# helemanc/audio-based-lyrics-matching

Measured on NVIDIA B200. Metric: similarity+MAP eval Gpairs/s at 1/2/4/8 B200 (roofline frac); MAP parity, higher is better.
Workload: dtype f16 tensor-core hi/lo split x3, f32 accumulate

## Files before the change

audio-based-lyrics-matching_b200/csrc/eval_sym_epilogue.cuh:

```cuda
#pragma once
#include "gemm_core.cuh"

namespace wealy {

struct EvalSymParams {
  const float4* lvl;
  const uint2* cinfo;
  const int* s_c;
  const int* s_i;
  const float* thr;
  unsigned int* hist;
  const unsigned char* dirty;
  int n_col_tiles;
  int n_row_blocks;
  unsigned int total_pairs;
  const float* beta;
  float* tk_val;
  int* tk_idx;
  int* tk_cnt;
  int tk_cap;
};

__device__ __forceinline__ unsigned bit_transpose32(unsigned x, int lane) {
#pragma unroll
  for (int s = 16; s >= 1; s >>= 1) {
    const unsigned mask = s == 16 ? 0x0000ffffu : s == 8 ? 0x00ff00ffu : s == 4 ? 0x0f0f0f0fu : s == 2 ? 0x33333333u : 0x55555555u;
    const unsigned y = __shfl_xor_sync(0xffffffffu, x, s);
    x = (lane & s) ? ((x & ~mask) | ((y >> s) & mask)) : ((x & mask) | ((y << s) & ~mask));
  }
  return x;
}

template <int kLv, int kQueueCapT = 256, int kCachePairsT = 4096, bool kTopk = false>
struct EvalSymEpi {
  static_assert(kLv >= 2 && kLv <= 4, "2..4 register levels");
  static_assert(!kTopk || kLv <= 3, "the top-k bound of the columns rides in the 4th threshold slot");
  using Params = EvalSymParams;
  static constexpr int kQueueCap = kQueueCapT;
  static constexpr int kCachePairs = kCachePairsT;
  static constexpr unsigned kGlobal = 0x80000000u;
  static constexpr int kOffQx = kQueueCap * 4;
  static constexpr int kOffQn = kOffQx + kQueueCap * 4;
  static constexpr int kStageCols = 16;
  static constexpr int kOffStage = kOffQn + kQueueCap * 4;
  static constexpr int kWarpScratchBytes = kOffStage + kStageCols * 32 * 4;
  static constexpr int kColSlots = 3;
  static constexpr int kLvlBytes = kTileN * 16;
  static constexpr int kInfoBytes = kTileN * 8;
  static constexpr int kColSlotBytes = kLvlBytes + kInfoBytes;
  static constexpr int kOffColSlots = (kCachePairs * 4 + 15) / 16 * 16;
  static constexpr int kCtaScratchBytes = kOffColSlots + kColSlots * kColSlotBytes;

  __device__ static __forceinline__ void col_bulk_src(const Params& p, int t, const void*& s0, const void*& s1) {
    s0 = p.lvl + (size_t)t * kTileN;
    s1 = p.cinfo + (size_t)t * kTileN;
  }

  struct RowState {
    float t[kLv];
    unsigned rc[kLv - 1];
    unsigned rinfo;
    int rpc;
    int qc, qi;
    unsigned off;
    int qn;
    int n_cached;
    unsigned base;
    int row_glob, row_ok, dirty;
    float beta;
  };

  __device__ static __forceinline__ float* q_val(const EpiCtx& c) { return reinterpret_cast<float*>(c.warp_scratch); }
  __device__ static __forceinline__ unsigned* q_idx(const EpiCtx& c) { return reinterpret_cast<unsigned*>(c.warp_scratch + kOffQx); }
  __device__ static __forceinline__ int* q_len(const EpiCtx& c) { return reinterpret_cast<int*>(c.warp_scratch + kOffQn); }
  __device__ static __forceinline__ float* stage(const EpiCtx& c) { return reinterpret_cast<float*>(c.warp_scratch + kOffStage); }
  __device__ static __forceinline__ float* thr_s(const EpiCtx& c) { return reinterpret_cast<float*>(c.cta_scratch); }

  __device__ static __forceinline__ float lvl_of(const float4& v, int j) {
    return j == 0 ? v.x : (j == 1 ? v.y : (j == 2 ? v.z : v.w));
  }

  __device__ static __forceinline__ void row_begin(const Params& p, RowState& st, int row, int part,
                                                   const GemmShape& sh, const EpiCtx& ctx) {
    (void)part;
    const float inf = __int_as_float(0x7f800000);
#pragma unroll
    for (int j = 0; j < kLv; ++j) st.t[j] = inf;
#pragma unroll
    for (int j = 0; j < kLv - 1; ++j) st.rc[j] = 0u;
    st.qc = st.qi = 0;
    st.off = 0u;
    st.beta = inf;
    int cnt = 0;
    const int srow = spread_sorted_of(row);
    st.row_ok = srow < sh.m_rows;
    if (st.row_ok) {
      const float4 v = __ldg(p.lvl + row);
#pragma unroll
      for (int j = 0; j < kLv; ++j) st.t[j] = lvl_of(v, j);
      const uint2 ci = __ldg(p.cinfo + row);
      st.off = ci.x;
      cnt = (int)ci.y;
      st.qc = __ldg(p.s_c + srow);
      st.qi = __ldg(p.s_i + srow);
      if constexpr (kTopk) st.beta = __ldg(p.beta + row);
    }
    st.qn = 0;
    st.row_glob = row;
    st.dirty = 0;
    st.base = __ldg(p.cinfo + ctx.row_base).x;
    const unsigned end = (ctx.row_base + ctx.row_span < sh.m_rows) ? __ldg(p.cinfo + ctx.row_base + ctx.row_span).x : p.total_pairs;
    const unsigned total = end - st.base;
    st.n_cached = (int)(total < (unsigned)kCachePairs ? total : (unsigned)kCachePairs);
    float* ts = thr_s(ctx);
    for (int i = ctx.tid; i < st.n_cached; i += ctx.nthreads) ts[i] = __ldg(p.thr + st.base + i);
    const unsigned rel = st.off - st.base;
    const bool cached = st.row_ok && rel + (unsigned)cnt <= (unsigned)st.n_cached;
    st.rinfo = cached ? (rel + kLv) : (kGlobal | (st.off + kLv));
    st.rpc = cnt - kLv;
    ptx::named_barrier_sync(1, ctx.nthreads);
  }

  __device__ static __forceinline__ int warp_incl_scan(int v, int lane) {
#pragma unroll
    for (int o = 1; o < 32; o <<= 1) {
      const int t = __shfl_up_sync(0xffffffffu, v, o);
      if (lane >= o) v += t;
    }
    return v;
  }

  struct Ent {
    float s;
    unsigned idx;
    int len;
    int cand;
    bool on;
    const float* tp;
  };
  __device__ static __forceinline__ void fetch(const Params& p, const EpiCtx& ctx, Ent& en, int r, int end) {
    en.on = r < end;
    en.s = en.on ? q_val(ctx)[r] : 0.f;
    en.idx = en.on ? q_idx(ctx)[r] : 0u;
    const int raw = en.on ? q_len(ctx)[r] : 0;
    en.len = max(raw, 0);
    en.cand = kTopk ? -1 - raw : -1;
    en.tp = (en.idx & kGlobal) ? (p.thr + (en.idx & ~kGlobal)) : (thr_s(ctx) + en.idx);
  }
  __device__ static __forceinline__ void count(const Params& p, const RowState& st, const EpiCtx& ctx, const Ent& en,
                                               int lb, int lane) {
    (void)ctx; (void)lane;
    if constexpr (kTopk) {
      if (en.cand >= 0) {
        if (en.on) {
          const int pos = atomicAdd(p.tk_cnt + en.idx, 1);
          if (pos < p.tk_cap) {
            p.tk_val[(size_t)en.idx * p.tk_cap + pos] = en.s;
            p.tk_idx[(size_t)en.idx * p.tk_cap + pos] = en.cand;
          }
        }
        return;
      }
    }
    const bool glob = (en.idx & kGlobal) != 0u;
    const unsigned slot = (en.idx & ~kGlobal) - 1u + (unsigned)lb + (glob ? 0u : st.base);
    if (en.on) atomicAdd(p.hist + slot, 1u);
  }

  __device__ static __forceinline__ void drain(const Params& p, RowState& st, const EpiCtx& ctx) {
    if (st.qn == 0) return;
    const int lane = (int)ptx::lane_id();
    __syncwarp();
    const int end = st.qn;
    for (int r0 = 0; r0 < end; r0 += 64) {
      Ent a, b;
      fetch(p, ctx, a, r0 + lane, end);
      fetch(p, ctx, b, r0 + 32 + lane, end);
      int loa = 0, hia = a.len, lob = 0, hib = b.len;
      while (loa < hia || lob < hib) {
        if (loa < hia) {
          const int mid = (loa + hia) >> 1;
          if (a.tp[mid] < a.s) loa = mid + 1; else hia = mid;
        }
        if (lob < hib) {
          const int mid = (lob + hib) >> 1;
          if (b.tp[mid] < b.s) lob = mid + 1; else hib = mid;
        }
      }
      count(p, st, ctx, a, loa, lane);
      if (r0 + 32 < end) count(p, st, ctx, b, lob, lane);
    }
    __syncwarp();
    st.qn = 0;
  }

  __device__ static __forceinline__ void push(const RowState& st, const EpiCtx& ctx, const uint32_t (&acc)[32], unsigned mr,
                                              unsigned mcq, const uint2* cinf, int pos, unsigned tkr = 0u, unsigned tkc = 0u,
                                              int col0 = 0) {
    float* qv = q_val(ctx);
    unsigned* qx = q_idx(ctx);
    int* ql = q_len(ctx);
    float* stg = stage(ctx) + (ptx::lane_id());
#pragma unroll
    for (int h = 0; h < 32 / kStageCols; ++h) {
      const unsigned sel = ((1u << kStageCols) - 1u) << (h * kStageCols);
      if (!__any_sync(0xffffffffu, ((mr | mcq | tkr | tkc) & sel) != 0u)) continue;
#pragma unroll
      for (int e = 0; e < kStageCols; ++e) stg[e * 32] = __uint_as_float(acc[h * kStageCols + e]);
      unsigned m = mr & sel;
      while (m) {
        const int e = __ffs(m) - 1;
        m &= m - 1;
        qv[pos] = stg[(e - h * kStageCols) * 32];
        qx[pos] = st.rinfo;
        ql[pos] = st.rpc;
        ++pos;
      }
      m = mcq & sel;
      while (m) {
        const int e = __ffs(m) - 1;
        m &= m - 1;
        const uint2 c = cinf[e];
        qv[pos] = stg[(e - h * kStageCols) * 32];
        qx[pos] = kGlobal | (c.x + kLv);
        ql[pos] = (int)c.y - kLv;
        ++pos;
      }
      if constexpr (kTopk) {
        m = tkr & sel;
        while (m) {
          const int e = __ffs(m) - 1;
          m &= m - 1;
          qv[pos] = stg[(e - h * kStageCols) * 32];
          qx[pos] = (unsigned)st.row_glob;
          ql[pos] = -1 - (col0 + e);
          ++pos;
        }
        m = tkc & sel;
        while (m) {
          const int e = __ffs(m) - 1;
          m &= m - 1;
          qv[pos] = stg[(e - h * kStageCols) * 32];
          qx[pos] = (unsigned)(col0 + e);
          ql[pos] = -1 - st.row_glob;
          ++pos;
        }
      }
      __syncwarp();
    }
  }

  __device__ static __forceinline__ void tile_begin(const Params& p, RowState& st, const GemmShape& sh,
                                                    const EpiCtx& ctx, int t) {
    (void)sh;
    st.dirty = 0;
    for (int rbi = ctx.row_base / kTileM; rbi < (ctx.row_base + ctx.row_span) / kTileM; ++rbi)
      st.dirty |= rbi < p.n_row_blocks ? (int)__ldg(p.dirty + (size_t)rbi * p.n_col_tiles + t) : 1;
  }

  __device__ static __forceinline__ void chunk32(const Params& p, RowState& st, int row, int col0,
                                                 const uint32_t (&acc)[32], const GemmShape& sh, const EpiCtx& ctx) {
    constexpr unsigned kFull = 0xffffffffu;
    const int lane = (int)ptx::lane_id();
    (void)row;
    const float4* lv = reinterpret_cast<const float4*>(ctx.col_slot) + (col0 & (kTileN - 1));
    const uint2* cinf = reinterpret_cast<const uint2*>(ctx.col_slot + kLvlBytes) + (col0 & (kTileN - 1));

    unsigned m[kLv], mc[kLv];
    unsigned tkr = 0u, tkc = 0u;
#pragma unroll
    for (int j = 0; j < kLv; ++j) m[j] = mc[j] = 0u;
#pragma unroll
    for (int e = 0; e < 32; ++e) {
      const float s = __uint_as_float(acc[e]);
      const float4 c = lv[e];
#pragma unroll
      for (int j = 0; j < kLv; ++j) {
        m[j] |= (s > st.t[j]) ? (1u << e) : 0u;
        mc[j] |= (s > lvl_of(c, j)) ? (1u << e) : 0u;
      }
      if constexpr (kTopk) {
        tkr |= (s > st.beta) ? (1u << e) : 0u;
        tkc |= (s > c.w) ? (1u << e) : 0u;
      }
    }
    if (st.dirty) {
      const int scol = spread_sorted_of(col0 + lane);
      const bool ok = scol < sh.n_cols;
      const int cc = ok ? __ldg(p.s_c + scol) : 0;
      const int ci = ok ? __ldg(p.s_i + scol) : 0;
      unsigned valid = 0u, validk = 0u;
#pragma unroll
      for (int e = 0; e < 32; ++e) {
        const int cce = __shfl_sync(kFull, cc, e);
        const int cie = __shfl_sync(kFull, ci, e);
        const int oke = __shfl_sync(kFull, (int)ok, e);
        valid |= (oke && cce != st.qc && cie != st.qi) ? (1u << e) : 0u;
        if constexpr (kTopk) validk |= (oke && cie != st.qi) ? (1u << e) : 0u;
      }
      const int d = st.row_glob - col0;
      const unsigned above = d < 0 ? 0xffffffffu : (d >= 31 ? 0u : (0xffffffffu << (d + 1)));
      valid &= above;
      validk &= above;
      if (!st.row_ok) valid = validk = 0u;
#pragma unroll
      for (int j = 0; j < kLv; ++j) {
        m[j] &= valid;
        mc[j] &= valid;
      }
      tkr &= validk;
      tkc &= validk;
    }
    if constexpr (kTopk) {
      if (!__any_sync(kFull, (m[0] | mc[0] | tkr | tkc) != 0u)) return;
    } else {
      if (!__any_sync(kFull, (m[0] | mc[0]) != 0u)) return;
    }

#pragma unroll
    for (int j = 0; j < kLv - 1; ++j) st.rc[j] += (unsigned)__popc(m[j] ^ m[j + 1]);
    if (__any_sync(kFull, (mc[0] ^ mc[kLv - 1]) != 0u)) {
      const unsigned coff = cinf[lane].x;
#pragma unroll
      for (int j = 0; j < kLv - 1; ++j) {
        const unsigned n = (unsigned)__popc(bit_transpose32(mc[j] ^ mc[j + 1], lane));
        if (n != 0u) atomicAdd(p.hist + coff + j, n);
      }
    }

    const unsigned dr = m[kLv - 1], dc = mc[kLv - 1];
    if (!__any_sync(kFull, (dr | dc | tkr | tkc) != 0u)) return;
    const int mine = __popc(dr) + __popc(dc) + __popc(tkr) + __popc(tkc);
    const int incl = warp_incl_scan(mine, lane);
    const int total = __shfl_sync(kFull, incl, 31);
    if (st.qn + total > kQueueCap) drain(p, st, ctx);
    if (total <= kQueueCap) {
      push(st, ctx, acc, dr, dc, cinf, st.qn + incl - mine, tkr, tkc, col0);
      st.qn += total;
    } else {
      constexpr int kBatchCols = kQueueCap / (kTopk ? 128 : 64);
      static_assert(kBatchCols >= 1 && 32 % kBatchCols == 0, "queue capacity: 64 (128 with top-k) .. 2048, a power of two");
#pragma unroll 1
      for (int g = 0; g < 32 / kBatchCols; ++g) {
        const unsigned sel = ((1u << kBatchCols) - 1u) << (kBatchCols * g);
        const int mine_g = __popc(dr & sel) + __popc(dc & sel) + __popc(tkr & sel) + __popc(tkc & sel);
        const int incl_g = warp_incl_scan(mine_g, lane);
        push(st, ctx, acc, dr & sel, dc & sel, cinf, incl_g - mine_g, tkr & sel, tkc & sel, col0);
        st.qn = __shfl_sync(kFull, incl_g, 31);
        drain(p, st, ctx);
      }
    }
  }

  __device__ static __forceinline__ void tile_end(const Params& p, RowState& st, const GemmShape&, const EpiCtx& ctx) {
    if (st.qn >= kQueueCap / 2) drain(p, st, ctx);
  }

  __device__ static __forceinline__ void row_end(const Params& p, RowState& st, int row, int part,
                                                 const GemmShape& sh, const EpiCtx& ctx) {
    (void)row; (void)part; (void)sh;
    drain(p, st, ctx);
    if (st.row_ok) {
#pragma unroll
      for (int j = 0; j < kLv - 1; ++j)
        if (st.rc[j] != 0u) atomicAdd(p.hist + st.off + j, st.rc[j]);
    }
    ptx::named_barrier_sync(1, ctx.nthreads);
  }
};

}
```

audio-based-lyrics-matching_b200/csrc/gemm_core2.cuh:

```cuda
#pragma once
#include "gemm_core.cuh"

namespace wealy {

template <int kPasses, int kBlockK, int kStages>
struct PairSmem {
  static constexpr int kSwizzle = kBlockK * 2;
  static constexpr int kTileBytes = kTileM * kBlockK * 2;
  static constexpr int kPlanes = kPasses == 3 ? 2 : 1;
  static constexpr int kStageBytes = kPlanes * 2 * kTileBytes;
  static constexpr int kBarBytes = 512;
  static constexpr int kCore = kStages * kStageBytes + kBarBytes;
  static constexpr int total(int epi_warps, int scratch_per_warp, int cta_scratch) {
    return kCore + epi_warps * scratch_per_warp + cta_scratch + 1024;
  }
};

template <class Epi, int kPasses, int kBlockK, int kEpiWarps, int kStages, bool kDynChunks = false>
__global__ void __cluster_dims__(2, 1, 1) __launch_bounds__(64 + kEpiWarps * 32, 1)
gemm_pair_kernel(const __grid_constant__ GemmTmaps tmaps, const GemmShape shape, const typename Epi::Params ep) {
  using SM = PairSmem<kPasses, kBlockK, kStages>;
  using CS = ColSlotTraits<Epi>;
  constexpr int kHalves = kEpiWarps / 4;
  constexpr int kColSlots = CS::kSlots;
#ifdef WEALY_LATE_RELEASE
  constexpr bool kEarlyRelease = false;
#else
  constexpr bool kEarlyRelease = true;
#endif
  static_assert(kEpiWarps == 8 || kEpiWarps == 12, "8 or 12 epilogue warps (2 or 3 per TMEM lane quadrant)");
  static_assert(kColSlots > 0 || !kDynChunks, "dynamic chunk claiming belongs to the symmetric evaluation epilogue");

  extern __shared__ uint8_t smem_raw[];
  uint8_t* smem = smem_raw + ((1024u - (ptx::smem_u32(smem_raw) & 1023u)) & 1023u);
  uint8_t* bar_base = smem + kStages * SM::kStageBytes;
  uint64_t* full_bar = reinterpret_cast<uint64_t*>(bar_base);
  uint64_t* empty_bar = full_bar + kStages;
  uint64_t* tmem_full = empty_bar + kStages;
  uint64_t* tmem_empty = tmem_full + 2;
  uint64_t* unit_full = tmem_empty + 2;
  uint64_t* unit_empty = unit_full + 2;
  uint64_t* col_full = unit_empty + 2;
  uint64_t* col_empty = col_full + (kColSlots > 0 ? kColSlots : 1);
  int* unit_slot = reinterpret_cast<int*>(col_empty + (kColSlots > 0 ? kColSlots : 1));
  uint32_t* tmem_slot = reinterpret_cast<uint32_t*>(unit_slot + 2);
  int* chunk_ctr = reinterpret_cast<int*>(tmem_slot + 2);
  static_assert((2 * kStages + 8 + 2 * (kColSlots > 0 ? kColSlots : 1)) * 8 + 16 + 32 <= SM::kBarBytes, "barrier area");
  constexpr int kChunksPerTile = kTileN / kChunkCols;
  uint8_t* scratch_base = bar_base + SM::kBarBytes;
  uint8_t* col_slots = scratch_base + kEpiWarps * Epi::kWarpScratchBytes + CS::kOffset;

  const int warp_idx = __shfl_sync(0xffffffffu, (int)(threadIdx.x >> 5), 0);
  const int lane = (int)ptx::lane_id();
  const uint32_t cta_rank = ptx::cluster_ctarank();
  const bool leader = cta_rank == 0;

  if (warp_idx == 0 && lane == 0) {
    ptx::prefetch_tensormap(&tmaps.a_hi);
    ptx::prefetch_tensormap(&tmaps.b_hi);
    if (kPasses == 3) {
      ptx::prefetch_tensormap(&tmaps.a_lo);
      ptx::prefetch_tensormap(&tmaps.b_lo);
    }
    for (int s = 0; s < kStages; ++s) {
      ptx::mbar_init(&full_bar[s], 1);
      ptx::mbar_init(&empty_bar[s], 1);
    }
    for (int a = 0; a < 2; ++a) {
      ptx::mbar_init(&tmem_full[a], 1);
      ptx::mbar_init(&tmem_empty[a], kDynChunks ? 2 * 4 * kChunksPerTile : 2 * kEpiWarps);
      ptx::mbar_init(&unit_full[a], 1);
      ptx::mbar_init(&unit_empty[a], 2 * kEpiWarps + 2);
    }
    for (int c = 0; c < kColSlots; ++c) {
      ptx::mbar_init(&col_full[c], 1);
      ptx::mbar_init(&col_empty[c], kDynChunks ? 4 * kChunksPerTile : kEpiWarps);
    }
    for (int k = 0; k < 8; ++k) chunk_ctr[k] = 0;
    ptx::fence_mbar_init();
  }
  if (warp_idx == 1) ptx::tmem_alloc_pair<512>(tmem_slot);
  ptx::tc_fence_before_sync();
  ptx::cluster_sync_all();
  ptx::tc_fence_after_sync();
  const uint32_t tmem_base = *tmem_slot;

  const int n_units = shape.n_row_blocks * shape.n_col_chunks;

  auto unit_tiles_c = [&](int u, int& S, int& t0, int& t1, int& chunk) {
    decode_unit(shape, u, chunk, S);
    t1 = min((chunk + 1) * shape.tiles_per_chunk, shape.n_col_tiles);
    t0 = shape.sym ? max(chunk * shape.tiles_per_chunk, S) : chunk * shape.tiles_per_chunk;
  };
  auto unit_tiles = [&](int u, int& S, int& t0, int& t1) {
    int chunk;
    unit_tiles_c(u, S, t0, t1, chunk);
  };

  if (warp_idx == 0) {
    if (lane == 0) {
      int stage = 0;
      uint32_t phase = 0;
      int us = 0;
      uint32_t uphase = 0;
      int cs = 0;
      uint32_t cphase = 0;
      const uint32_t leader_full0 = ptx::map_to_cta(&full_bar[0], 0);
      const uint32_t peer_unit_full0 = ptx::map_to_cta(&unit_full[0], 1);
      const uint32_t peer_unit_slot0 = ptx::map_to_cta(&unit_slot[0], 1);
      const uint32_t leader_unit_empty0 = ptx::map_to_cta(&unit_empty[0], 0);
      const uint32_t peer_chunk_ctr0 = ptx::map_to_cta(&chunk_ctr[0], 1);
      while (true) {
        int u;
        if (leader) {
          ptx::mbar_wait_cluster(&unit_empty[us], uphase ^ 1u);
          u = atomicAdd(shape.unit_counter, 1);
          if (u >= n_units) u = -1;
          unit_slot[us] = u;
          ptx::st_cluster_u32(peer_unit_slot0 + 4u * us, (uint32_t)u);
          if constexpr (kDynChunks) {
            for (int k = 0; k < 4; ++k) {
              chunk_ctr[us * 4 + k] = 0;
              ptx::st_cluster_u32(peer_chunk_ctr0 + 4u * (us * 4 + k), 0u);
            }
          }
          ptx::mbar_arrive(&unit_full[us]);
          ptx::mbar_arrive_cluster(peer_unit_full0 + 8u * us);
        } else {
          ptx::mbar_wait_cluster(&unit_full[us], uphase);
          u = unit_slot[us];
          ptx::mbar_arrive_cluster_relaxed(leader_unit_empty0 + 8u * us);
        }
        if (++us == 2) { us = 0; uphase ^= 1u; }
        if (u < 0) break;
        int rb, t0, t1;
        unit_tiles(u, rb, t0, t1);
        for (int t = t0; t < t1; ++t) {
          if constexpr (kColSlots > 0) {
            ptx::mbar_wait(&col_empty[cs], cphase ^ 1u);
            const void *s0, *s1;
            Epi::col_bulk_src(ep, t, s0, s1);
            uint8_t* dst = col_slots + cs * CS::kBytes;
            ptx::mbar_expect_tx(&col_full[cs], CS::kBytes);
            ptx::bulk_load(dst, s0, Epi::kLvlBytes, &col_full[cs]);
            ptx::bulk_load(dst + Epi::kLvlBytes, s1, CS::kBytes - Epi::kLvlBytes, &col_full[cs]);
            if (++cs == kColSlots) { cs = 0; cphase ^= 1u; }
          }
          for (int kb = 0; kb < shape.k_blocks; ++kb) {
            ptx::mbar_wait_cluster(&empty_bar[stage], phase ^ 1u);
            uint8_t* st = smem + stage * SM::kStageBytes;
            if (leader) ptx::mbar_expect_tx(&full_bar[stage], 2 * SM::kStageBytes);
            const uint32_t fb = leader_full0 + 8u * stage;
            const int brow = t * kTileN + (int)cta_rank * kTileM;
            const int arow = (shape.sym & 2) ? rb * 2 * kTileM + (int)cta_rank : rb * 2 * kTileM + (int)cta_rank * kTileM;
            ptx::tma_load_2d_pair(st, &tmaps.a_hi, fb, kb * kBlockK, arow, ptx::kEvictLast);
            ptx::tma_load_2d_pair(st + SM::kPlanes * SM::kTileBytes, &tmaps.b_hi, fb, kb * kBlockK, brow, ptx::kEvictNormal);
            if (kPasses == 3) {
              ptx::tma_load_2d_pair(st + SM::kTileBytes, &tmaps.a_lo, fb, kb * kBlockK, arow, ptx::kEvictLast);
              ptx::tma_load_2d_pair(st + 3 * SM::kTileBytes, &tmaps.b_lo, fb, kb * kBlockK, brow, ptx::kEvictNormal);
            }
            if (++stage == kStages) { stage = 0; phase ^= 1u; }
          }
        }
      }
    }
  } else if (warp_idx == 1) {
    if (lane == 0 && leader) {
      constexpr uint32_t idesc = ptx::make_idesc_f16(2 * kTileM, kTileN, false);
      int stage = 0;
      uint32_t phase = 0;
      int acc = 0;
      uint32_t acc_phase = 0;
      int us = 0;
      uint32_t uphase = 0;
#ifdef WEALY_PROFILE_WAITS
      long long w_unit = 0, w_acc = 0, w_full = 0, n_tiles_done = 0;
      const long long t_begin = clock64();
#define WEALY_TIMED(var, stmt) { const long long _t = clock64(); stmt; var += clock64() - _t; }
#else
#define WEALY_TIMED(var, stmt) stmt;
#endif
      while (true) {
        WEALY_TIMED(w_unit, ptx::mbar_wait(&unit_full[us], uphase))
        const int u = unit_slot[us];
        ptx::mbar_arrive(&unit_empty[us]);
        if (++us == 2) { us = 0; uphase ^= 1u; }
        if (u < 0) break;
        int rb, t0, t1;
        unit_tiles(u, rb, t0, t1);
        for (int t = t0; t < t1; ++t) {
          WEALY_TIMED(w_acc, ptx::mbar_wait_cluster(&tmem_empty[acc], acc_phase ^ 1u))
          ptx::tc_fence_after_sync();
#ifdef WEALY_PROFILE_WAITS
          ++n_tiles_done;
#endif
          const uint32_t d_tmem = tmem_base + (uint32_t)(acc * kTileN);
          for (int kb = 0; kb < shape.k_blocks; ++kb) {
            WEALY_TIMED(w_full, ptx::mbar_wait_cluster(&full_bar[stage], phase))
            ptx::tc_fence_after_sync();
            const uint32_t st = ptx::smem_u32(smem + stage * SM::kStageBytes);
            const uint64_t a_hi = ptx::make_smem_desc<SM::kSwizzle>(st);
            const uint64_t a_lo = ptx::make_smem_desc<SM::kSwizzle>(st + SM::kTileBytes);
            const uint64_t b_hi = ptx::make_smem_desc<SM::kSwizzle>(st + SM::kPlanes * SM::kTileBytes);
            const uint64_t b_lo = ptx::make_smem_desc<SM::kSwizzle>(st + 3 * SM::kTileBytes);
#pragma unroll
            for (int kk = 0; kk < kBlockK / kUmmaK; ++kk) {
              const uint64_t adv = (uint64_t)((kk * kUmmaK * 2) >> 4);
              ptx::umma_f16_pair(d_tmem, a_hi + adv, b_hi + adv, idesc, (uint32_t)((kb | kk) != 0));
              if (kPasses == 3) {
                ptx::umma_f16_pair(d_tmem, a_hi + adv, b_lo + adv, idesc, 1u);
                ptx::umma_f16_pair(d_tmem, a_lo + adv, b_hi + adv, idesc, 1u);
              }
            }
            ptx::umma_commit_pair(&empty_bar[stage]);
            if (kb == shape.k_blocks - 1) ptx::umma_commit_pair(&tmem_full[acc]);
            if (++stage == kStages) { stage = 0; phase ^= 1u; }
          }
          if (++acc == 2) { acc = 0; acc_phase ^= 1u; }
        }
      }
#ifdef WEALY_PROFILE_WAITS
      if ((blockIdx.x % 37) == 0)
        printf("wealy waits: cta %d tiles %lld total %lld cyc | wait unit %lld acc(epilogue) %lld full(tma) %lld\n", (int)blockIdx.x,
               n_tiles_done, clock64() - t_begin, w_unit, w_acc, w_full);
#endif
    }
  } else {
    const int ew = warp_idx - 2;
    const int quad = warp_idx & 3;
    const int half = ew >> 2;
    const int row_in_tile = quad * 32 + lane;
    int acc = 0;
    uint32_t acc_phase = 0;
    int us = 0;
    uint32_t uphase = 0;
    int cs = 0;
    uint32_t cphase = 0;
    const uint32_t leader_unit_empty0 = ptx::map_to_cta(&unit_empty[0], 0);
    const uint32_t leader_tmem_empty0 = ptx::map_to_cta(&tmem_empty[0], 0);
    unsigned tile_seq = 0;
    int pending_slot = -1;
    while (true) {
      ptx::mbar_wait_cluster_warp(&unit_full[us], uphase);
      const int u = unit_slot[us];
      const int us_claim = us;
      __syncwarp();
      if constexpr (kDynChunks) {
        if (pending_slot >= 0 && lane == 0) ptx::mbar_arrive_cluster_relaxed(leader_unit_empty0 + 8u * pending_slot);
        pending_slot = us;
      } else {
        if (lane == 0) ptx::mbar_arrive_cluster_relaxed(leader_unit_empty0 + 8u * us);
      }
      if (++us == 2) { us = 0; uphase ^= 1u; }
      if (u < 0) break;
      int rb, t0, t1, chunk;
      unit_tiles_c(u, rb, t0, t1, chunk);
      if (t0 >= t1) continue;
      const int row = (shape.sym & 2) ? rb * 2 * kTileM + 2 * row_in_tile + (int)cta_rank
                                      : rb * 2 * kTileM + (int)cta_rank * kTileM + row_in_tile;
      const int part = chunk * kHalves + half;
      typename Epi::RowState rs;
      EpiCtx ctx;
      ctx.warp_scratch = scratch_base + ew * Epi::kWarpScratchBytes;
      ctx.cta_scratch = scratch_base + kEpiWarps * Epi::kWarpScratchBytes;
      ctx.tid = ew * 32 + lane;
      ctx.nthreads = kEpiWarps * 32;
      ctx.row_base = (shape.sym & 2) ? rb * 2 * kTileM : rb * 2 * kTileM + (int)cta_rank * kTileM;
      ctx.row_span = (shape.sym & 2) ? 2 * kTileM : kTileM;
      ctx.first_col = t0 * kTileN + half * kChunkCols;
      ctx.col_step = kHalves * kChunkCols;
      ctx.col_slot = nullptr;
      Epi::row_begin(ep, rs, row, part, shape, ctx);
      if constexpr (kDynChunks) {
        const int n_tiles = t1 - t0;
        const int total = n_tiles * kChunksPerTile;
        int* ctr = &chunk_ctr[us_claim * 4 + quad];
        int cur = -1, a_cur = 0, c_cur = 0;
        while (true) {
          int g = 0;
          if (lane == 0) g = atomicAdd(ctr, 1);
          g = __shfl_sync(0xffffffffu, g, 0);
          if (g >= total) break;
          const int tile = g / kChunksPerTile, c = g - tile * kChunksPerTile;
          if (tile != cur) {
            if (cur >= 0) Epi::tile_end(ep, rs, shape, ctx);
            const unsigned seq = tile_seq + (unsigned)tile;
            a_cur = (int)(seq & 1u);
            c_cur = (int)(seq % (unsigned)kColSlots);
            ptx::mbar_wait_warp(&col_full[c_cur], (seq / (unsigned)kColSlots) & 1u);
            ctx.col_slot = col_slots + c_cur * CS::kBytes;
            Epi::tile_begin(ep, rs, shape, ctx, t0 + tile);
            ptx::mbar_wait_cluster_warp(&tmem_full[a_cur], (seq >> 1) & 1u);
            ptx::tc_fence_after_sync();
            cur = tile;
          }
          const uint32_t taddr = tmem_base + ((uint32_t)(quad * 32) << 16) + (uint32_t)(a_cur * kTileN);
          uint32_t v[32];
          ptx::tmem_ld_32x32(taddr + (uint32_t)(c * kChunkCols), v);
          ptx::tmem_ld_wait();
          ptx::tc_fence_before_sync();
          __syncwarp();
          if (kEarlyRelease && lane == 0) ptx::mbar_arrive_cluster_relaxed(leader_tmem_empty0 + 8u * a_cur);
          Epi::chunk32(ep, rs, row, (t0 + tile) * kTileN + c * kChunkCols, v, shape, ctx);
          __syncwarp();
          if (lane == 0) {
            if (!kEarlyRelease) ptx::mbar_arrive_cluster_relaxed(leader_tmem_empty0 + 8u * a_cur);
            ptx::mbar_arrive(&col_empty[c_cur]);
          }
        }
        if (cur >= 0) Epi::tile_end(ep, rs, shape, ctx);
        tile_seq += (unsigned)n_tiles;
      } else {
      for (int t = t0; t < t1; ++t) {
        if constexpr (kColSlots > 0) {
          ptx::mbar_wait_warp(&col_full[cs], cphase);
          ctx.col_slot = col_slots + cs * CS::kBytes;
        }
        Epi::tile_begin(ep, rs, shape, ctx, t);
        ptx::mbar_wait_cluster_warp(&tmem_full[acc], acc_phase);
        ptx::tc_fence_after_sync();
        const uint32_t taddr = tmem_base + ((uint32_t)(quad * 32) << 16) + (uint32_t)(acc * kTileN);
#pragma unroll 1
        for (int c = half; c < kTileN / kChunkCols; c += kHalves) {
          uint32_t v[32];
          ptx::tmem_ld_32x32(taddr + (uint32_t)(c * kChunkCols), v);
          ptx::tmem_ld_wait();
          Epi::chunk32(ep, rs, row, t * kTileN + c * kChunkCols, v, shape, ctx);
        }
        ptx::tc_fence_before_sync();
        __syncwarp();
        if (lane == 0) {
          ptx::mbar_arrive_cluster_relaxed(leader_tmem_empty0 + 8u * acc);
          if constexpr (kColSlots > 0) ptx::mbar_arrive(&col_empty[cs]);
        }
        if (++acc == 2) { acc = 0; acc_phase ^= 1u; }
        if constexpr (kColSlots > 0) {
          if (++cs == kColSlots) { cs = 0; cphase ^= 1u; }
        }
        Epi::tile_end(ep, rs, shape, ctx);
      }
      }
      Epi::row_end(ep, rs, row, part, shape, ctx);
    }
  }

  ptx::tc_fence_before_sync();
  ptx::cluster_sync_all();
  if (warp_idx == 1) {
    ptx::tc_fence_after_sync();
    ptx::tmem_dealloc_pair<512>(tmem_base);
  }
  release_unit_counter(shape);
}

}
```

audio-based-lyrics-matching_b200/csrc/ptx.cuh:

```cuda
#pragma once
#include <cstdint>
#include <cuda.h>
#include <cuda_runtime.h>

namespace wealy {
namespace ptx {

__device__ __forceinline__ uint32_t smem_u32(const void* p) {
  return static_cast<uint32_t>(__cvta_generic_to_shared(p));
}

__device__ __forceinline__ uint32_t lane_id() {
  uint32_t l;
  asm volatile("mov.u32 %0, %%laneid;" : "=r"(l));
  return l;
}

__device__ __forceinline__ void mbar_init(uint64_t* bar, uint32_t count) {
  asm volatile("mbarrier.init.shared::cta.b64 [%0], %1;" ::"r"(smem_u32(bar)), "r"(count));
}

__device__ __forceinline__ void fence_mbar_init() {
  asm volatile("fence.mbarrier_init.release.cluster;" ::: "memory");
}

__device__ __forceinline__ void fence_proxy_async() {
  asm volatile("fence.proxy.async.shared::cta;" ::: "memory");
}

__device__ __forceinline__ void mbar_expect_tx(uint64_t* bar, uint32_t bytes) {
  asm volatile("mbarrier.arrive.expect_tx.shared::cta.b64 _, [%0], %1;" ::"r"(smem_u32(bar)), "r"(bytes)
               : "memory");
}

__device__ __forceinline__ void mbar_arrive(uint64_t* bar) {
  asm volatile("mbarrier.arrive.shared::cta.b64 _, [%0];" ::"r"(smem_u32(bar)) : "memory");
}

#ifndef WEALY_WAIT_HINT_NS
#define WEALY_WAIT_HINT_NS 1000
#endif
#ifndef WEALY_WAIT_ALL_LANES
#define WEALY_WAIT_LANE0
#endif

__device__ __forceinline__ bool mbar_try_wait(uint64_t* bar, uint32_t parity) {
  uint32_t ok;
#if WEALY_WAIT_HINT_NS > 0
  asm volatile(
      "{\n"
      ".reg .pred P;\n"
      "mbarrier.try_wait.parity.shared::cta.b64 P, [%1], %2, %3;\n"
      "selp.u32 %0, 1, 0, P;\n"
      "}\n"
      : "=r"(ok)
      : "r"(smem_u32(bar)), "r"(parity), "r"((uint32_t)WEALY_WAIT_HINT_NS)
      : "memory");
#else
  asm volatile(
      "{\n"
      ".reg .pred P;\n"
      "mbarrier.try_wait.parity.shared::cta.b64 P, [%1], %2;\n"
      "selp.u32 %0, 1, 0, P;\n"
      "}\n"
      : "=r"(ok)
      : "r"(smem_u32(bar)), "r"(parity)
      : "memory");
#endif
  return ok != 0;
}

#ifndef WEALY_DEADLOCK_CYCLES
#define WEALY_DEADLOCK_CYCLES (4000000000ll)
#endif

__device__ __forceinline__ void mbar_wait(uint64_t* bar, uint32_t parity) {
  if (mbar_try_wait(bar, parity)) return;
  const long long t0 = clock64();
  int polls = 0;
  while (!mbar_try_wait(bar, parity)) {
    if ((++polls & 63) == 0 && clock64() - t0 > WEALY_DEADLOCK_CYCLES) {
      printf("wealy: mbarrier deadlock block=%d thread=%d bar=0x%x parity=%u\n", (int)blockIdx.x,
             (int)threadIdx.x, smem_u32(bar), parity);
      __trap();
    }
  }
}

__device__ __forceinline__ void mbar_wait_warp(uint64_t* bar, uint32_t parity) {
#ifdef WEALY_WAIT_LANE0
  if (lane_id() == 0) mbar_wait(bar, parity);
  __syncwarp();
#else
  mbar_wait(bar, parity);
#endif
}

__device__ __forceinline__ void named_barrier_sync(int id, int nthreads) {
  asm volatile("bar.sync %0, %1;" ::"r"(id), "r"(nthreads) : "memory");
}

__device__ __forceinline__ void prefetch_tensormap(const CUtensorMap* m) {
  asm volatile("prefetch.tensormap [%0];" ::"l"(reinterpret_cast<uint64_t>(m)) : "memory");
}

__device__ __forceinline__ void tma_load_2d(void* smem_dst, const CUtensorMap* m, uint64_t* bar, int32_t c0,
                                            int32_t c1, uint64_t cache_policy) {
  asm volatile(
      "cp.async.bulk.tensor.2d.shared::cluster.global.mbarrier::complete_tx::bytes.L2::cache_hint"
      " [%0], [%1, {%3, %4}], [%2], %5;"
      ::"r"(smem_u32(smem_dst)), "l"(reinterpret_cast<uint64_t>(m)), "r"(smem_u32(bar)), "r"(c0), "r"(c1),
        "l"(cache_policy)
      : "memory");
}

__device__ __forceinline__ void bulk_load(void* smem_dst, const void* gsrc, uint32_t bytes, uint64_t* bar) {
  asm volatile(
      "cp.async.bulk.shared::cluster.global.mbarrier::complete_tx::bytes [%0], [%1], %2, [%3];"
      ::"r"(smem_u32(smem_dst)), "l"(reinterpret_cast<uint64_t>(gsrc)), "r"(bytes), "r"(smem_u32(bar))
      : "memory");
}

constexpr uint64_t kEvictNormal = 0x1000000000000000ull;
constexpr uint64_t kEvictFirst = 0x12F0000000000000ull;
constexpr uint64_t kEvictLast = 0x14F0000000000000ull;

template <uint32_t kCols>
__device__ __forceinline__ void tmem_alloc(uint32_t* smem_result) {
  static_assert(kCols >= 32 && kCols <= 512 && (kCols & (kCols - 1)) == 0, "TMEM columns: power of two in [32,512]");
  asm volatile("tcgen05.alloc.cta_group::1.sync.aligned.shared::cta.b32 [%0], %1;" ::"r"(smem_u32(smem_result)),
               "n"(kCols)
               : "memory");
  asm volatile("tcgen05.relinquish_alloc_permit.cta_group::1.sync.aligned;" ::: "memory");
}

template <uint32_t kCols>
__device__ __forceinline__ void tmem_dealloc(uint32_t tmem_addr) {
  asm volatile("tcgen05.dealloc.cta_group::1.sync.aligned.b32 %0, %1;" ::"r"(tmem_addr), "n"(kCols) : "memory");
}

__device__ __forceinline__ void tc_fence_before_sync() {
  asm volatile("tcgen05.fence::before_thread_sync;" ::: "memory");
}
__device__ __forceinline__ void tc_fence_after_sync() {
  asm volatile("tcgen05.fence::after_thread_sync;" ::: "memory");
}

__device__ __forceinline__ void umma_f16(uint32_t tmem_d, uint64_t desc_a, uint64_t desc_b, uint32_t idesc,
                                         uint32_t accumulate) {
  asm volatile(
      "{\n"
      ".reg .pred p;\n"
      "setp.ne.b32 p, %4, 0;\n"
      "tcgen05.mma.cta_group::1.kind::f16 [%0], %1, %2, %3, p;\n"
      "}\n"
      ::"r"(tmem_d), "l"(desc_a), "l"(desc_b), "r"(idesc), "r"(accumulate)
      : "memory");
}

__device__ __forceinline__ void umma_commit(uint64_t* bar) {
  asm volatile("tcgen05.commit.cta_group::1.mbarrier::arrive::one.shared::cluster.b64 [%0];" ::"r"(smem_u32(bar))
               : "memory");
}

__device__ __forceinline__ void tmem_ld_32x32(uint32_t taddr, uint32_t (&v)[32]) {
  asm volatile(
      "tcgen05.ld.sync.aligned.32x32b.x32.b32 "
      "{%0, %1, %2, %3, %4, %5, %6, %7, %8, %9, %10, %11, %12, %13, %14, %15, "
      "%16, %17, %18, %19, %20, %21, %22, %23, %24, %25, %26, %27, %28, %29, %30, %31}, [%32];"
      : "=r"(v[0]), "=r"(v[1]), "=r"(v[2]), "=r"(v[3]), "=r"(v[4]), "=r"(v[5]), "=r"(v[6]), "=r"(v[7]), "=r"(v[8]),
        "=r"(v[9]), "=r"(v[10]), "=r"(v[11]), "=r"(v[12]), "=r"(v[13]), "=r"(v[14]), "=r"(v[15]), "=r"(v[16]),
        "=r"(v[17]), "=r"(v[18]), "=r"(v[19]), "=r"(v[20]), "=r"(v[21]), "=r"(v[22]), "=r"(v[23]), "=r"(v[24]),
        "=r"(v[25]), "=r"(v[26]), "=r"(v[27]), "=r"(v[28]), "=r"(v[29]), "=r"(v[30]), "=r"(v[31])
      : "r"(taddr)
      : "memory");
}

__device__ __forceinline__ void tmem_ld_wait() { asm volatile("tcgen05.wait::ld.sync.aligned;" ::: "memory"); }


__device__ __forceinline__ uint32_t cluster_ctarank() {
  uint32_t r;
  asm volatile("mov.u32 %0, %%cluster_ctarank;" : "=r"(r));
  return r;
}
__device__ __forceinline__ uint32_t cluster_id_x() {
  uint32_t r;
  asm volatile("mov.u32 %0, %%clusterid.x;" : "=r"(r));
  return r;
}
__device__ __forceinline__ uint32_t n_clusters_x() {
  uint32_t r;
  asm volatile("mov.u32 %0, %%nclusterid.x;" : "=r"(r));
  return r;
}
__device__ __forceinline__ void cluster_sync_all() {
  asm volatile("barrier.cluster.arrive.release.aligned;\n\tbarrier.cluster.wait.acquire.aligned;" ::: "memory");
}
__device__ __forceinline__ uint32_t map_to_cta(const void* p, uint32_t rank) {
  uint32_t r;
  asm volatile("mapa.shared::cluster.u32 %0, %1, %2;" : "=r"(r) : "r"(smem_u32(p)), "r"(rank));
  return r;
}
__device__ __forceinline__ void mbar_arrive_cluster(uint32_t cluster_addr) {
  asm volatile("mbarrier.arrive.release.cluster.shared::cluster.b64 _, [%0];" ::"r"(cluster_addr) : "memory");
}
__device__ __forceinline__ void mbar_arrive_cluster_relaxed(uint32_t cluster_addr) {
  asm volatile("mbarrier.arrive.relaxed.cluster.shared::cluster.b64 _, [%0];" ::"r"(cluster_addr) : "memory");
}
__device__ __forceinline__ void st_cluster_u32(uint32_t cluster_addr, uint32_t v) {
  asm volatile("st.shared::cluster.u32 [%0], %1;" ::"r"(cluster_addr), "r"(v) : "memory");
}
__device__ __forceinline__ void mbar_wait_cluster(uint64_t* bar, uint32_t parity) {
  const long long t0 = clock64();
  int polls = 0;
  while (true) {
    uint32_t ok;
    asm volatile(
        "{\n"
        ".reg .pred P;\n"
        "mbarrier.try_wait.parity.acquire.cluster.shared::cta.b64 P, [%1], %2, %3;\n"
        "selp.u32 %0, 1, 0, P;\n"
        "}\n"
        : "=r"(ok)
        : "r"(smem_u32(bar)), "r"(parity), "r"((uint32_t)(WEALY_WAIT_HINT_NS > 0 ? WEALY_WAIT_HINT_NS : 1))
        : "memory");
    if (ok) return;
    if ((++polls & 63) == 0 && clock64() - t0 > WEALY_DEADLOCK_CYCLES) {
      printf("wealy: cluster mbarrier deadlock block=%d thread=%d bar=0x%x parity=%u\n", (int)blockIdx.x,
             (int)threadIdx.x, smem_u32(bar), parity);
      __trap();
    }
  }
}

__device__ __forceinline__ void mbar_wait_cluster_warp(uint64_t* bar, uint32_t parity) {
  if (lane_id() == 0) mbar_wait_cluster(bar, parity);
  __syncwarp();
}

__device__ __forceinline__ void tma_load_2d_pair(void* smem_dst, const CUtensorMap* m, uint32_t leader_bar_addr, int32_t c0,
                                                 int32_t c1, uint64_t cache_policy) {
  asm volatile(
      "cp.async.bulk.tensor.2d.cta_group::2.shared::cluster.global.mbarrier::complete_tx::bytes.L2::cache_hint"
      " [%0], [%1, {%3, %4}], [%2], %5;"
      ::"r"(smem_u32(smem_dst)), "l"(reinterpret_cast<uint64_t>(m)), "r"(leader_bar_addr), "r"(c0), "r"(c1),
        "l"(cache_policy)
      : "memory");
}

template <uint32_t kCols>
__device__ __forceinline__ void tmem_alloc_pair(uint32_t* smem_result) {
  asm volatile("tcgen05.alloc.cta_group::2.sync.aligned.shared::cta.b32 [%0], %1;" ::"r"(smem_u32(smem_result)), "n"(kCols)
               : "memory");
  asm volatile("tcgen05.relinquish_alloc_permit.cta_group::2.sync.aligned;" ::: "memory");
}
template <uint32_t kCols>
__device__ __forceinline__ void tmem_dealloc_pair(uint32_t tmem_addr) {
  asm volatile("tcgen05.dealloc.cta_group::2.sync.aligned.b32 %0, %1;" ::"r"(tmem_addr), "n"(kCols) : "memory");
}

__device__ __forceinline__ void umma_f16_pair(uint32_t tmem_d, uint64_t desc_a, uint64_t desc_b, uint32_t idesc,
                                              uint32_t accumulate) {
  asm volatile(
      "{\n"
      ".reg .pred p;\n"
      "setp.ne.b32 p, %4, 0;\n"
      "tcgen05.mma.cta_group::2.kind::f16 [%0], %1, %2, %3, p;\n"
      "}\n"
      ::"r"(tmem_d), "l"(desc_a), "l"(desc_b), "r"(idesc), "r"(accumulate)
      : "memory");
}
__device__ __forceinline__ void umma_commit_pair(uint64_t* bar) {
  asm volatile(
      "tcgen05.commit.cta_group::2.mbarrier::arrive::one.shared::cluster.multicast::cluster.b64 [%0], %1;"
      ::"r"(smem_u32(bar)), "h"((uint16_t)3)
      : "memory");
}

template <int kSwizzleBytes>
__device__ __forceinline__ uint64_t make_smem_desc(uint32_t smem_addr) {
  static_assert(kSwizzleBytes == 128 || kSwizzleBytes == 64 || kSwizzleBytes == 32, "swizzle span");
  constexpr uint64_t layout = kSwizzleBytes == 128 ? 2ull : (kSwizzleBytes == 64 ? 4ull : 6ull);
  constexpr uint64_t sbo = (8ull * kSwizzleBytes) >> 4;
  return (uint64_t)((smem_addr & 0x3FFFFu) >> 4) | (1ull << 16) | (sbo << 32) | (1ull << 46) | (layout << 61);
}

__host__ __device__ constexpr uint32_t make_idesc_f16(int m, int n, bool bf16) {
  return (1u << 4) | ((bf16 ? 1u : 0u) << 7) | ((bf16 ? 1u : 0u) << 10) | ((uint32_t)(n >> 3) << 17) |
         ((uint32_t)(m >> 4) << 24);
}

}
}
```

Measured before the change: 427.0.

## Compute upper threshold levels lazily only for elements passing level zero

The epilogue chunk now compares each accumulator only against level-0 row and column thresholds (plus the top-k bounds), using explicit shared-memory scalar loads instead of float4 loads. Upper-level masks are computed afterwards, and only when some lane has a level-0 hit: a full dense pass when a lane has many hits, otherwise a sparse walk over the set bits through the staging buffer. This cuts comparison work and register pressure in the common case where few elements pass level zero. Epilogue waits on cluster barriers also gain a __nanosleep back-off after the first failed poll, and an optional profiling census is added behind a macro. The sleep may add wake-up latency on the epilogue's critical path.

```diff
diff --git a/audio-based-lyrics-matching_b200/csrc/eval_sym_epilogue.cuh b/audio-based-lyrics-matching_b200/csrc/eval_sym_epilogue.cuh
--- a/audio-based-lyrics-matching_b200/csrc/eval_sym_epilogue.cuh
+++ b/audio-based-lyrics-matching_b200/csrc/eval_sym_epilogue.cuh
@@ -76,6 +76,12 @@
   __device__ static __forceinline__ float* stage(const EpiCtx& c) { return reinterpret_cast<float*>(c.warp_scratch + kOffStage); }
   __device__ static __forceinline__ float* thr_s(const EpiCtx& c) { return reinterpret_cast<float*>(c.cta_scratch); }
 
+  __device__ static __forceinline__ float lds_f32(const float* p) {
+    float v;
+    asm volatile("ld.shared.f32 %0, [%1];" : "=f"(v) : "r"(ptx::smem_u32(p)));
+    return v;
+  }
+
   __device__ static __forceinline__ float lvl_of(const float4& v, int j) {
     return j == 0 ? v.x : (j == 1 ? v.y : (j == 2 ? v.z : v.w));
   }
@@ -258,6 +264,82 @@
       st.dirty |= rbi < p.n_row_blocks ? (int)__ldg(p.dirty + (size_t)rbi * p.n_col_tiles + t) : 1;
   }
 
+#ifdef WEALY_PROFILE_EPI
+  __device__ static __forceinline__ void census_chunk(unsigned pm) {
+    const bool cold = !__any_sync(0xffffffffu, pm != 0u);
+    if (ptx::lane_id() == 0) {
+      ptx::census_add(ptx::census::kChunks, 1ull);
+      if (cold) ptx::census_add(ptx::census::kCold, 1ull);
+    }
+  }
+  __device__ static __forceinline__ void census_levels(unsigned hot) {
+    if (ptx::lane_id() == 0) {
+      ptx::census_add(ptx::census::kHot + (int)hot, 1ull);
+      if (hot > (unsigned)kWalkMaxBits) ptx::census_add(ptx::census::kDenseUpper, 1ull);
+    }
+  }
+  __device__ static __forceinline__ void census_reach(const unsigned (&m)[kLv], const unsigned (&mc)[kLv]) {
+#pragma unroll
+    for (int j = 0; j < kLv; ++j) {
+      const unsigned n = __reduce_add_sync(0xffffffffu, (unsigned)(__popc(m[j]) + __popc(mc[j])));
+      if (ptx::lane_id() == 0) ptx::census_add(ptx::census::kReach + j, n);
+    }
+  }
+#endif
+
+  static constexpr int kWalkMaxBits = 12;
+  __device__ static __forceinline__ void upper_levels(const RowState& st, const uint32_t (&acc)[32], const float4* lv,
+                                                      const EpiCtx& ctx, unsigned (&m)[kLv], unsigned (&mc)[kLv]) {
+    constexpr unsigned kFull = 0xffffffffu;
+    const unsigned pm = m[0] | mc[0];
+    const unsigned hot = __reduce_max_sync(kFull, (unsigned)__popc(pm));
+#ifdef WEALY_PROFILE_EPI
+    census_levels(hot);
+#endif
+    if (hot > (unsigned)kWalkMaxBits) {
+#pragma unroll
+      for (int e = 0; e < 32; ++e) {
+        const float s = __uint_as_float(acc[e]);
+        const float4 c = lv[e];
+#pragma unroll
+        for (int j = 1; j < kLv; ++j) {
+          m[j] |= (s > st.t[j]) ? (1u << e) : 0u;
+          mc[j] |= (s > lvl_of(c, j)) ? (1u << e) : 0u;
+        }
+      }
+#pragma unroll
+      for (int j = 1; j < kLv; ++j) {
+        m[j] &= m[0];
+        mc[j] &= mc[0];
+      }
+    } else if (hot != 0u) {
+      float* stg = stage(ctx) + ptx::lane_id();
+#pragma unroll
+      for (int h = 0; h < 32 / kStageCols; ++h) {
+        const unsigned sel = ((1u << kStageCols) - 1u) << (h * kStageCols);
+        if (!__any_sync(kFull, (pm & sel) != 0u)) continue;
+#pragma unroll
+        for (int e = 0; e < kStageCols; ++e) stg[e * 32] = __uint_as_float(acc[h * kStageCols + e]);
+        unsigned b = pm & sel;
+        while (b) {
+          const int e = __ffs(b) - 1;
+          b &= b - 1;
+          const float s = stg[(e - h * kStageCols) * 32];
+          const float4 c = lv[e];
+          const unsigned bit = 1u << e;
+#pragma unroll
+          for (int j = 1; j < kLv; ++j) {
+            m[j] |= (s > st.t[j]) ? bit : 0u;
+            mc[j] |= (s > lvl_of(c, j)) ? bit : 0u;
+          }
+        }
+      }
+    }
+#ifdef WEALY_PROFILE_EPI
+    census_reach(m, mc);
+#endif
+  }
+
   __device__ static __forceinline__ void chunk32(const Params& p, RowState& st, int row, int col0,
                                                  const uint32_t (&acc)[32], const GemmShape& sh, const EpiCtx& ctx) {
     constexpr unsigned kFull = 0xffffffffu;
@@ -273,15 +355,11 @@
 #pragma unroll
     for (int e = 0; e < 32; ++e) {
       const float s = __uint_as_float(acc[e]);
-      const float4 c = lv[e];
-#pragma unroll
-      for (int j = 0; j < kLv; ++j) {
-        m[j] |= (s > st.t[j]) ? (1u << e) : 0u;
-        mc[j] |= (s > lvl_of(c, j)) ? (1u << e) : 0u;
-      }
+      m[0] |= (s > st.t[0]) ? (1u << e) : 0u;
+      mc[0] |= (s > lds_f32(&lv[e].x)) ? (1u << e) : 0u;
       if constexpr (kTopk) {
         tkr |= (s > st.beta) ? (1u << e) : 0u;
-        tkc |= (s > c.w) ? (1u << e) : 0u;
+        tkc |= (s > lds_f32(&lv[e].w)) ? (1u << e) : 0u;
       }
     }
     if (st.dirty) {
@@ -303,19 +381,20 @@
       valid &= above;
       validk &= above;
       if (!st.row_ok) valid = validk = 0u;
-#pragma unroll
-      for (int j = 0; j < kLv; ++j) {
-        m[j] &= valid;
-        mc[j] &= valid;
-      }
+      m[0] &= valid;
+      mc[0] &= valid;
       tkr &= validk;
       tkc &= validk;
     }
+#ifdef WEALY_PROFILE_EPI
+    census_chunk(m[0] | mc[0]);
+#endif
     if constexpr (kTopk) {
       if (!__any_sync(kFull, (m[0] | mc[0] | tkr | tkc) != 0u)) return;
     } else {
       if (!__any_sync(kFull, (m[0] | mc[0]) != 0u)) return;
     }
+    upper_levels(st, acc, lv, ctx, m, mc);
 
 #pragma unroll
     for (int j = 0; j < kLv - 1; ++j) st.rc[j] += (unsigned)__popc(m[j] ^ m[j + 1]);
diff --git a/audio-based-lyrics-matching_b200/csrc/gemm_core2.cuh b/audio-based-lyrics-matching_b200/csrc/gemm_core2.cuh
--- a/audio-based-lyrics-matching_b200/csrc/gemm_core2.cuh
+++ b/audio-based-lyrics-matching_b200/csrc/gemm_core2.cuh
@@ -147,7 +147,7 @@
             if (++cs == kColSlots) { cs = 0; cphase ^= 1u; }
           }
           for (int kb = 0; kb < shape.k_blocks; ++kb) {
-            ptx::mbar_wait_cluster(&empty_bar[stage], phase ^ 1u);
+            ptx::mbar_wait_cluster(&empty_bar[stage], phase ^ 1u, ptx::kWaitTmaEmpty);
             uint8_t* st = smem + stage * SM::kStageBytes;
             if (leader) ptx::mbar_expect_tx(&full_bar[stage], 2 * SM::kStageBytes);
             const uint32_t fb = leader_full0 + 8u * stage;
@@ -189,14 +189,14 @@
         int rb, t0, t1;
         unit_tiles(u, rb, t0, t1);
         for (int t = t0; t < t1; ++t) {
-          WEALY_TIMED(w_acc, ptx::mbar_wait_cluster(&tmem_empty[acc], acc_phase ^ 1u))
+          WEALY_TIMED(w_acc, ptx::mbar_wait_cluster(&tmem_empty[acc], acc_phase ^ 1u, ptx::kWaitMmaTmemEmpty))
           ptx::tc_fence_after_sync();
 #ifdef WEALY_PROFILE_WAITS
           ++n_tiles_done;
 #endif
           const uint32_t d_tmem = tmem_base + (uint32_t)(acc * kTileN);
           for (int kb = 0; kb < shape.k_blocks; ++kb) {
-            WEALY_TIMED(w_full, ptx::mbar_wait_cluster(&full_bar[stage], phase))
+            WEALY_TIMED(w_full, ptx::mbar_wait_cluster(&full_bar[stage], phase, ptx::kWaitMmaFull))
             ptx::tc_fence_after_sync();
             const uint32_t st = ptx::smem_u32(smem + stage * SM::kStageBytes);
             const uint64_t a_hi = ptx::make_smem_desc<SM::kSwizzle>(st);
@@ -241,7 +241,7 @@
     unsigned tile_seq = 0;
     int pending_slot = -1;
     while (true) {
-      ptx::mbar_wait_cluster_warp(&unit_full[us], uphase);
+      ptx::mbar_wait_cluster_warp<true>(&unit_full[us], uphase, ptx::kWaitEpiUnit);
       const int u = unit_slot[us];
       const int us_claim = us;
       __syncwarp();
@@ -290,7 +290,7 @@
             ptx::mbar_wait_warp(&col_full[c_cur], (seq / (unsigned)kColSlots) & 1u);
             ctx.col_slot = col_slots + c_cur * CS::kBytes;
             Epi::tile_begin(ep, rs, shape, ctx, t0 + tile);
-            ptx::mbar_wait_cluster_warp(&tmem_full[a_cur], (seq >> 1) & 1u);
+            ptx::mbar_wait_cluster_warp<true>(&tmem_full[a_cur], (seq >> 1) & 1u, ptx::kWaitEpiTmemFull);
             ptx::tc_fence_after_sync();
             cur = tile;
           }
@@ -317,7 +317,7 @@
           ctx.col_slot = col_slots + cs * CS::kBytes;
         }
         Epi::tile_begin(ep, rs, shape, ctx, t);
-        ptx::mbar_wait_cluster_warp(&tmem_full[acc], acc_phase);
+        ptx::mbar_wait_cluster_warp<true>(&tmem_full[acc], acc_phase, ptx::kWaitEpiTmemFull);
         ptx::tc_fence_after_sync();
         const uint32_t taddr = tmem_base + ((uint32_t)(quad * 32) << 16) + (uint32_t)(acc * kTileN);
 #pragma unroll 1
@@ -351,6 +351,9 @@
     ptx::tmem_dealloc_pair<512>(tmem_base);
   }
   release_unit_counter(shape);
+#ifdef WEALY_PROFILE_EPI
+  ptx::census_finish();
+#endif
 }
 
 }
diff --git a/audio-based-lyrics-matching_b200/csrc/ptx.cuh b/audio-based-lyrics-matching_b200/csrc/ptx.cuh
--- a/audio-based-lyrics-matching_b200/csrc/ptx.cuh
+++ b/audio-based-lyrics-matching_b200/csrc/ptx.cuh
@@ -211,33 +211,107 @@
 __device__ __forceinline__ void st_cluster_u32(uint32_t cluster_addr, uint32_t v) {
   asm volatile("st.shared::cluster.u32 [%0], %1;" ::"r"(cluster_addr), "r"(v) : "memory");
 }
-__device__ __forceinline__ void mbar_wait_cluster(uint64_t* bar, uint32_t parity) {
+enum WaitRole : int {
+  kWaitAny = -1,
+  kWaitEpiTmemFull = 0,
+  kWaitEpiUnit,
+  kWaitMmaFull,
+  kWaitMmaTmemEmpty,
+  kWaitTmaEmpty,
+  kWaitRoles
+};
+
+#ifdef WEALY_PROFILE_EPI
+namespace census {
+enum : int {
+  kChunks = 0,
+  kCold,
+  kDenseUpper,
+  kHot,
+  kReach = kHot + 33,
+  kWaits = kReach + 4,
+  kPolls = kWaits + kWaitRoles,
+  kN = kPolls + kWaitRoles
+};
+}
+__device__ unsigned long long g_census[census::kN];
+__device__ unsigned int g_census_done;
+__device__ __forceinline__ void census_add(int k, unsigned long long v) {
+  if (v != 0ull) atomicAdd(&g_census[k], v);
+}
+#endif
+
+__device__ __forceinline__ bool mbar_try_wait_cluster(uint64_t* bar, uint32_t parity) {
+  uint32_t ok;
+  asm volatile(
+      "{\n"
+      ".reg .pred P;\n"
+      "mbarrier.try_wait.parity.acquire.cluster.shared::cta.b64 P, [%1], %2, %3;\n"
+      "selp.u32 %0, 1, 0, P;\n"
+      "}\n"
+      : "=r"(ok)
+      : "r"(smem_u32(bar)), "r"(parity), "r"((uint32_t)(WEALY_WAIT_HINT_NS > 0 ? WEALY_WAIT_HINT_NS : 1))
+      : "memory");
+  return ok != 0;
+}
+
+#ifndef WEALY_IDLE_SLEEP_NS
+#define WEALY_IDLE_SLEEP_NS 256
+#endif
+
+template <bool kIdle = false>
+__device__ __forceinline__ void mbar_wait_cluster(uint64_t* bar, uint32_t parity, int role = kWaitAny) {
+  (void)role;
+  if (mbar_try_wait_cluster(bar, parity)) return;
   const long long t0 = clock64();
-  int polls = 0;
+  int polls = 1;
   while (true) {
-    uint32_t ok;
-    asm volatile(
-        "{\n"
-        ".reg .pred P;\n"
-        "mbarrier.try_wait.parity.acquire.cluster.shared::cta.b64 P, [%1], %2, %3;\n"
-        "selp.u32 %0, 1, 0, P;\n"
-        "}\n"
-        : "=r"(ok)
-        : "r"(smem_u32(bar)), "r"(parity), "r"((uint32_t)(WEALY_WAIT_HINT_NS > 0 ? WEALY_WAIT_HINT_NS : 1))
-        : "memory");
-    if (ok) return;
+    if constexpr (kIdle) __nanosleep(WEALY_IDLE_SLEEP_NS);
+    if (mbar_try_wait_cluster(bar, parity)) break;
     if ((++polls & 63) == 0 && clock64() - t0 > WEALY_DEADLOCK_CYCLES) {
       printf("wealy: cluster mbarrier deadlock block=%d thread=%d bar=0x%x parity=%u\n", (int)blockIdx.x,
              (int)threadIdx.x, smem_u32(bar), parity);
       __trap();
     }
   }
-}
-
-__device__ __forceinline__ void mbar_wait_cluster_warp(uint64_t* bar, uint32_t parity) {
-  if (lane_id() == 0) mbar_wait_cluster(bar, parity);
+#ifdef WEALY_PROFILE_EPI
+  if (role >= 0) {
+    census_add(census::kWaits + role, 1ull);
+    census_add(census::kPolls + role, (unsigned long long)polls);
+  }
+#endif
+}
+
+template <bool kIdle = false>
+__device__ __forceinline__ void mbar_wait_cluster_warp(uint64_t* bar, uint32_t parity, int role = kWaitAny) {
+  if (lane_id() == 0) mbar_wait_cluster<kIdle>(bar, parity, role);
   __syncwarp();
 }
+
+#ifdef WEALY_PROFILE_EPI
+__device__ __forceinline__ void census_finish() {
+  __syncthreads();
+  if (threadIdx.x != 0) return;
+  __threadfence();
+  if (atomicAdd(&g_census_done, 1u) != gridDim.x - 1) return;
+  __threadfence();
+  volatile unsigned long long* c = g_census;
+  printf("wealy epi census: warp-chunks %llu | no level-0 bit %llu | dense upper levels %llu\n", c[census::kChunks],
+         c[census::kCold], c[census::kDenseUpper]);
+  printf("wealy epi census: elements above level 0/1/2/3 %llu %llu %llu %llu (of %llu)\n", c[census::kReach],
+         c[census::kReach + 1], c[census::kReach + 2], c[census::kReach + 3], c[census::kChunks] * 2048ull);
+  for (int b = 0; b <= 32; ++b)
+    if (c[census::kHot + b] != 0ull) printf("wealy epi census: hottest lane %2d level-0 bits: %llu warp-chunks\n", b, c[census::kHot + b]);
+  const char* names[kWaitRoles] = {"epilogue tmem_full", "epilogue unit mailbox", "mma full_bar", "mma tmem_empty",
+                                   "tma empty_bar"};
+  for (int r = 0; r < kWaitRoles; ++r)
+    printf("wealy epi census: %-21s waits that polled more than once %llu, failed polls %llu\n", names[r],
+           c[census::kWaits + r], c[census::kPolls + r]);
+  for (int k = 0; k < census::kN; ++k) c[k] = 0ull;
+  g_census_done = 0u;
+  __threadfence();
+}
+#endif
 
 __device__ __forceinline__ void tma_load_2d_pair(void* smem_dst, const CUtensorMap* m, uint32_t leader_bar_addr, int32_t c0,
                                                  int32_t c1, uint64_t cache_policy) {
```

Result: no change. 426.7 (median of 6 runs) (-0.1%).
